# gizatechxyz/LuminAIR

Hardware: AMD Instinct MI355X
Metric: proofs/sec, 2^20-row Add trace (higher is better)
Workload: dtype u32 (M31/QM31 field arithmetic)

## Files before the change

### luminair_amd/csrc/fft_fixed.h

```cpp
#pragma once
#include "kernels.h"

namespace lmn {

bool launch_fft_fixed_pass(bool inverse, uint32_t* data, uint64_t col_stride, const uint32_t* src, uint64_t src_stride, int lo,
                           int rbits, int cb, int log_n, const TwPtrs& tw, uint32_t scale_log, int ncols, int cpb,
                           uint32_t h_off, int xcd_swizzle, bool zero_extended_top, lmn_stream_t s);
bool launch_interp_extend_fixed(uint32_t* coeffs, uint64_t coeff_stride, uint32_t* lde, uint64_t lde_stride, int log_n,
                                const TwPtrs& itw, const TwPtrs& tw_ext, int ncols, lmn_stream_t s);
bool launch_fft_rows_fixed(uint32_t* coeffs, uint64_t col_stride, const uint32_t* rows, uint64_t n_rows, int ncols, int log_n,
                           const PadRow& pad, uint32_t* bad_flag, uint32_t bad_value, const TwPtrs& itw, lmn_stream_t s);

}
```

### luminair_amd/csrc/fft_fixed.hip

```cpp
#include "fft_fixed.h"

#include <algorithm>

#include "issue_phases.h"
#include "launch_util.h"

namespace lmn {

LMN_HD constexpr uint32_t fx_pad(uint32_t e) { return e + (e >> 5); }

#if !defined(LMN_EMU) && !defined(LMN_BATCH)
#define LMN_BOUNDS(n) __launch_bounds__(n)
#else
#define LMN_BOUNDS(n)
#endif

struct GTile {
#if defined(__HIP_DEVICE_COMPILE__) && !defined(LMN_EMU)
  __amdgpu_buffer_rsrc_t r;
#else
  uint32_t* p;
#endif
};
LMN_D GTile gtile(const uint32_t* p) {
// ... 110 lines not shown
        d[k] = a[k] - x[k];
        d2[k] = d[k] + P31;
      }
      LMN_PHASE_PORT0();
#pragma unroll
      for (int k = 0; k < NB; ++k) {
        const int j = ((k >> r) << (r + 1)) | (k & ((1 << r) - 1));
        v[j] = u[k] < u2[k] ? u[k] : u2[k];
        v[j | (1 << r)] = d[k] < d2[k] ? d[k] : d2[k];
      }
    }
  }
  LMN_PHASE_ANY();
}

template <int R, int r, int HB>
LMN_D void fx_load_twiddles(uint32_t (&t2)[(1 << R) - 1], const uint32_t* const (&twd)[MAX_LOG], int layer0, uint32_t H,
                            uint32_t mhigh) {
  const uint32_t* __restrict__ t = twd[layer0 + r];
  const uint32_t hb = (H << (HB - r - 1)) + (mhigh << (R - 1 - r));
  LMN_ASSUME(hb < (1u << 28));
  fx_load_run<(1 << (R - 1 - r))>(t + hb, &t2[fx_tw_at<R>(r)]);
  if constexpr (r + 1 < R) fx_load_twiddles<R, r + 1, HB>(t2, twd, layer0, H, mhigh);
}

LMN_D uint32_t m_rot(uint32_t x, uint32_t e) {
#if defined(__HIP_DEVICE_COMPILE__) && !defined(LMN_EMU)
  return __builtin_amdgcn_alignbit(x, x + x, 32u - e) & P31;
#else
  return (uint32_t)((((uint64_t)x << e) | ((uint64_t)x >> (31u - e))) & P31);
#endif
}

template <int RBITS_, int CB_, bool LO0_>
struct FxShape {
  static constexpr int RBITS = RBITS_, CB = CB_, TB = RBITS_ + CB_;
  static constexpr bool LO0 = LO0_;
  static constexpr int NT = 1 << (TB - 4);
  static constexpr int NST = (RBITS + 3) / 4;
  static constexpr int R(int k) {
    int f = 0, r = 0;
    for (int i = 0; i <= k; ++i) {
      r = (RBITS - f + (NST - i) - 1) / (NST - i);
      f += r;
    }
    return r;
  }
  static constexpr int F(int k) {
    int f = 0;
    for (int i = 0; i < k; ++i) f += R(i);
    return f;
  }
  static constexpr uint32_t LDS_WORDS = (1u << TB) + ((1u << TB) >> 5) + 1u;
};

template <int R, bool INV, int P, class S, bool FG, bool TG, bool KEEP, bool ZX = false>
LMN_D void fx_stage(const uint32_t* sm_in, uint32_t* sm_out, uint32_t* tdst, const uint32_t* tsrc,
                    int lo, uint32_t H, const uint32_t* const (&twd)[MAX_LOG], uint32_t scale_log, uint32_t* keep, uint32_t tid) {
  constexpr int TB = S::TB, CB = S::CB, RBITS = S::RBITS;
  constexpr bool LO0 = S::LO0;
  constexpr uint32_t NG = 1u << (TB - R);
  constexpr uint32_t NT = (uint32_t)S::NT;
  constexpr int ITER = (int)(NG / NT);
  constexpr int L0 = P - CB;
  constexpr uint32_t cmask = (1u << CB) - 1u;
  static_assert(NG >= NT && P >= CB && P + R <= TB, "stage outside the tile");
#pragma unroll
  for (int it = 0; it < ITER; ++it) {
    const uint32_t g = tid + (uint32_t)it * NT;
    const uint32_t e0 = ((g >> P) << (P + R)) | (g & ((1u << P) - 1u));
    const uint32_t mhigh = e0 >> (P + R);
    uint32_t t2[(1 << R) - 1];
    fx_load_twiddles<R, 0, RBITS - L0>(t2, twd, (LO0 ? 0 : lo) + L0, H, mhigh);
    uint32_t v[1 << R];
    const uint32_t off0 = LO0 ? e0 : (((e0 >> CB) << lo) + (e0 & cmask));
    LMN_ASSUME(off0 < 0x10000000u);
    const int gshift = LO0 ? P : (P - CB + lo);
    if constexpr (FG) {
      if constexpr (LO0 && P == 0 && R >= 2) {
        fx_load_run<(1 << R)>(tsrc + e0, v);
      } else if constexpr (ZX) {
        static_assert(!INV && P + R == TB, "zero extension: forward transform, top stage");
        const GTile gt = gtile(tsrc);
#pragma unroll
        for (int j = 0; j < (1 << (R - 1)); ++j) {
          v[j] = gtile_load(gt, off0, (uint32_t)j << gshift);
          v[j + (1 << (R - 1))] = v[j];
        }
      } else {
        const GTile gt = gtile(tsrc);
#pragma unroll
        for (int j = 0; j < (1 << R); ++j) v[j] = gtile_load(gt, off0, (uint32_t)j << gshift);
      }
    } else {
      const uint32_t pb = fx_pad(e0);
#pragma unroll
      for (int j = 0; j < (1 << R); ++j) v[j] = sm_in[pb + fx_pad((uint32_t)j << P)];
    }
    fx_butterflies<R, INV, ZX>(v, t2);
    if constexpr (TG) {
      if constexpr (INV) {
        if (scale_log != 0u) {
#pragma unroll
          for (int j = 0; j < (1 << R); ++j) v[j] = m_rot(v[j], scale_log);
        }
      }
      if constexpr (LO0 && P == 0 && R >= 2) {
#if !defined(LMN_EMU)
// ... 36 lines not shown
}

struct TwD {
  const uint32_t* l[MAX_LOG];
};
static TwD doubled(const TwPtrs& tw) {
  TwD t{};
  for (int i = 0; i < MAX_LOG; ++i) t.l[i] = tw.d[i];
  return t;
}

template <bool INV, int RBITS, int CB, bool LO0, bool ZX = false>
LMN_KERNEL LMN_BOUNDS((FxShape<RBITS, CB, LO0>::NT))
k_fft_fx(uint32_t* data, uint64_t col_stride, const uint32_t* src, uint64_t src_stride, int lo_arg, TwD tw, uint32_t scale_log,
         int ncols, int cpb, uint32_t h_off, int xcd_swizzle) {
  using S = FxShape<RBITS, CB, LO0>;
  LMN_DYN_SMEM(uint32_t, sm);
  const int lo = LO0 ? 0 : lo_arg;
  uint32_t tile = blockIdx.x;
  if (xcd_swizzle && (gridDim.x & 7u) == 0u) tile = (blockIdx.x & 7u) * (gridDim.x >> 3) + (blockIdx.x >> 3);
  const uint32_t q = tile & ((1u << (lo - CB)) - 1u);
  const uint32_t Hl = tile >> (lo - CB);
  const uint64_t base = ((uint64_t)Hl << (lo + RBITS)) + ((uint64_t)q << CB);
  const uint32_t H = Hl + h_off;
  for (int cc = 0; cc < cpb; ++cc) {
    const int c = (int)blockIdx.y * cpb + cc;
    if (c >= ncols) break;
    uint32_t* col = data + (uint64_t)c * col_stride + base;
    const uint32_t* scol = src + (uint64_t)c * src_stride + base;
    fx_steps<S, INV, 0, true, true, false, ZX>(sm, sm, col, scol, lo, H, tw.l, scale_log, nullptr, threadIdx.x);
  }
}

template <int RBITS>
LMN_KERNEL LMN_BOUNDS((FxShape<RBITS, 4, false>::NT))
k_fft_interp_extend_fx(uint32_t* coeffs, uint64_t coeff_stride, uint32_t* lde, uint64_t lde_stride, TwD itw, TwD tw,
                       uint32_t scale_log) {
  using S = FxShape<RBITS, 4, false>;
  constexpr int LO = 12;
  LMN_DYN_SMEM(uint32_t, sm);
  uint32_t* A = sm;
  uint32_t* B = sm + S::LDS_WORDS;
  uint32_t tile = blockIdx.x;
  if ((gridDim.x & 7u) == 0u) tile = (blockIdx.x & 7u) * (gridDim.x >> 3) + (blockIdx.x >> 3);
  const uint64_t base = (uint64_t)tile << 4;
  const uint64_t n_words = 1ull << (LO + RBITS);
  uint32_t* ccol = coeffs + (uint64_t)blockIdx.y * coeff_stride + base;
  uint32_t* lcol = lde + (uint64_t)blockIdx.y * lde_stride + base;
  fx_steps<S, true, 0, true, true, true>(B, B, ccol, ccol, LO, 0u, itw.l, scale_log, A, threadIdx.x);
  for (uint32_t h = 0; h < 2; ++h)
    fx_steps<S, false, 0, false, true, false>(A, B, lcol + h * n_words, nullptr, LO, h, tw.l, 0u, nullptr, threadIdx.x);
}

template <int COLS>
LMN_KERNEL LMN_BOUNDS((COLS / 2) * 256)
k_fft_rows_fx(uint32_t* coeffs, uint64_t col_stride, const uint32_t* __restrict__ rows, uint64_t n_rows, int ncols, PadRow pad,
              uint32_t* __restrict__ bad_flag, uint32_t bad_value, TwD itw, uint32_t n_groups) {
  using S = FxShape<12, 0, true>;
  constexpr uint32_t NT = (uint32_t)S::NT, TILE = 1u << 12, GROUPS = COLS / 2;
  static_assert(NT == 256, "one lane group per tile");
  LMN_DYN_SMEM(uint32_t, sm);
  uint32_t tile = blockIdx.x / n_groups, ygrp = blockIdx.x % n_groups;
  if ((gridDim.x & 7u) == 0u && ((gridDim.x / n_groups) & 7u) == 0u) {
    const uint32_t x = blockIdx.x & 7u, sq = blockIdx.x >> 3;
    tile = (sq / n_groups) * 8u + x;
    ygrp = sq % n_groups;
  }
  const int c0 = (int)ygrp * COLS;
  const int ncb = ncols - c0 < COLS ? ncols - c0 : COLS;
  const uint64_t row0 = (uint64_t)tile << 12;
  {
    constexpr int BATCH = 8;
    constexpr uint32_t CELLS = TILE * COLS, STEP = GROUPS * NT;
    for (uint32_t k0 = threadIdx.x; k0 < CELLS; k0 += BATCH * STEP) {
      uint32_t v[BATCH];
#pragma unroll
      for (int j = 0; j < BATCH; ++j) {
        const uint32_t k = k0 + (uint32_t)j * STEP;
        const uint32_t r = k / COLS, c = k % COLS;
        const uint64_t gr = row0 + r;
        v[j] = 0u;
        if ((int)c < ncb) v[j] = gr < n_rows ? rows[gr * (uint64_t)ncols + (uint32_t)c0 + c] : pad.v[(uint32_t)c0 + c];
      }
#pragma unroll
      for (int j = 0; j < BATCH; ++j) {
        const uint32_t k = k0 + (uint32_t)j * STEP;
        const uint32_t r = k / COLS, c = k % COLS;
        if (v[j] >= P31) *bad_flag = bad_value;
        if ((int)c < ncb) sm[c * S::LDS_WORDS + fx_pad(r)] = v[j];
      }
    }
  }
  __syncthreads();
#if defined(__HIP_DEVICE_COMPILE__) && !defined(LMN_EMU)
  const uint32_t grp = __builtin_amdgcn_readfirstlane(threadIdx.x / NT);
#else
  const uint32_t grp = threadIdx.x / NT;
#endif
  const uint32_t tid = threadIdx.x % NT;
  for (int round = 0; round * (int)GROUPS < COLS; ++round) {
    const int cl = round * (int)GROUPS + (int)grp;
    const bool active = cl < ncb;
    uint32_t* t = sm + (uint32_t)(active ? cl : 0) * S::LDS_WORDS;
    uint32_t* col = coeffs + (uint64_t)(c0 + (active ? cl : 0)) * col_stride + row0;
    fx_steps<S, true, 0, false, true, false>(t, t, col, nullptr, 0, tile, itw.l, 0u, nullptr, tid, active);
  }
}

template <int COLS>
static void launch_rows_fx(uint32_t* coeffs, uint64_t col_stride, const uint32_t* rows, uint64_t n_rows, int ncols, int log_n,
                           const PadRow& pad, uint32_t* bad_flag, uint32_t bad_value, const TwPtrs& itw, lmn_stream_t s) {
  using S = FxShape<12, 0, true>;
  const size_t smem = (size_t)4 * COLS * S::LDS_WORDS;
  const uint32_t n_groups = (uint32_t)((ncols + COLS - 1) / COLS);
#if !defined(LMN_EMU) && !defined(LMN_BATCH)
  if (smem > 64 * 1024) allow_big_lds((const void*)k_fft_rows_fx<COLS>, 160 * 1024);
#endif
  LMN_LAUNCH((k_fft_rows_fx<COLS>), dim3((1u << (log_n - 12)) * n_groups), dim3((COLS / 2) * 256), smem, s, coeffs, col_stride,
             rows, n_rows, ncols, pad, bad_flag, bad_value, doubled(itw), n_groups);
}

bool launch_fft_rows_fixed(uint32_t* coeffs, uint64_t col_stride, const uint32_t* rows, uint64_t n_rows, int ncols, int log_n,
                           const PadRow& pad, uint32_t* bad_flag, uint32_t bad_value, const TwPtrs& itw, lmn_stream_t s) {
  static const bool off = env_set("LMN_NO_FFT_FIXED");
  if (off || !itw.d[0] || log_n < 13 || ncols < 1 || ncols > 32) return false;
  const int cols = env_int("LMN_ROWS_FX_COLS", 8);
  if (cols == 4)
    launch_rows_fx<4>(coeffs, col_stride, rows, n_rows, ncols, log_n, pad, bad_flag, bad_value, itw, s);
  else
    launch_rows_fx<8>(coeffs, col_stride, rows, n_rows, ncols, log_n, pad, bad_flag, bad_value, itw, s);
  return true;
}

template <bool INV, int RBITS, int CB, bool LO0, bool ZX = false>
static void launch_fx(uint32_t* data, uint64_t col_stride, const uint32_t* src, uint64_t src_stride, int lo, int log_n,
                      const TwPtrs& tw, uint32_t scale_log, int ncols, int cpb, uint32_t h_off, int xcd, lmn_stream_t s) {
  using S = FxShape<RBITS, CB, LO0>;
  const unsigned tiles = 1u << (log_n - S::TB);
  const size_t smem = (size_t)4 * S::LDS_WORDS;
#if !defined(LMN_EMU) && !defined(LMN_BATCH)
  if (smem > 64 * 1024) allow_big_lds((const void*)k_fft_fx<INV, RBITS, CB, LO0, ZX>, 160 * 1024);
#endif
  LMN_LAUNCH((k_fft_fx<INV, RBITS, CB, LO0, ZX>), dim3(tiles, (unsigned)((ncols + cpb - 1) / cpb)), dim3(S::NT), smem, s, data,
             col_stride, src, src_stride, lo, doubled(tw), scale_log, ncols, cpb, h_off, xcd);
}

template <bool INV>
static bool dispatch_fx(uint32_t* data, uint64_t col_stride, const uint32_t* src, uint64_t src_stride, int lo, int rbits, int cb,
                        int log_n, const TwPtrs& tw, uint32_t scale_log, int ncols, int cpb, uint32_t h_off, int xcd,
                        bool zext, lmn_stream_t s) {
#define LMN_FX_CASE(RB, CBV, L0V)                                                                                            \
  if constexpr (!INV && !L0V) {                                                                                              \
    if (zext) {                                                                                                              \
      launch_fx<INV, RB, CBV, L0V, true>(data, col_stride, src, src_stride, lo, log_n, tw, scale_log, ncols, cpb, h_off, xcd, \
                                         s);                                                                                 \
      return true;                                                                                                           \
    }                                                                                                                        \
  }                                                                                                                          \
  if (zext) return false;                                                                                                    \
  launch_fx<INV, RB, CBV, L0V>(data, col_stride, src, src_stride, lo, log_n, tw, scale_log, ncols, cpb, h_off, xcd, s);      \
  return true
  if (lo == 0 && cb == 0) {
    if (rbits == 12) { LMN_FX_CASE(12, 0, true); }
// ... 3 lines not shown
    switch (rbits) {
      case 5: LMN_FX_CASE(5, 5, false);
      case 6: LMN_FX_CASE(6, 5, false);
      case 7: LMN_FX_CASE(7, 5, false);
      default: return false;
    }
  }
  if (cb == 4 && lo >= 4) {
    switch (rbits) {
      case 6: LMN_FX_CASE(6, 4, false);
      case 7: LMN_FX_CASE(7, 4, false);
      case 8: LMN_FX_CASE(8, 4, false);
      case 9: LMN_FX_CASE(9, 4, false);
      case 10: LMN_FX_CASE(10, 4, false);
      default: return false;
    }
  }
  return false;
#undef LMN_FX_CASE
}

bool launch_fft_fixed_pass(bool inverse, uint32_t* data, uint64_t col_stride, const uint32_t* src, uint64_t src_stride, int lo,
                           int rbits, int cb, int log_n, const TwPtrs& tw, uint32_t scale_log, int ncols, int cpb,
                           uint32_t h_off, int xcd_swizzle, bool zero_extended_top, lmn_stream_t s) {
  static const bool off = env_set("LMN_NO_FFT_FIXED");
  if (off || !tw.d[0]) return false;
  if (zero_extended_top && (inverse || lo + rbits != log_n)) return false;
  return inverse ? dispatch_fx<true>(data, col_stride, src, src_stride, lo, rbits, cb, log_n, tw, scale_log, ncols, cpb, h_off,
                                     xcd_swizzle, false, s)
                 : dispatch_fx<false>(data, col_stride, src, src_stride, lo, rbits, cb, log_n, tw, scale_log, ncols, cpb, h_off,
                                      xcd_swizzle, zero_extended_top, s);
}

template <int RBITS>
static void launch_ie(uint32_t* coeffs, uint64_t coeff_stride, uint32_t* lde, uint64_t lde_stride, const TwPtrs& itw,
                      const TwPtrs& tw_ext, uint32_t scale_log, int ncols, lmn_stream_t s) {
  using S = FxShape<RBITS, 4, false>;
  const size_t smem = (size_t)8 * S::LDS_WORDS;
#if !defined(LMN_EMU) && !defined(LMN_BATCH)
  if (smem > 64 * 1024) allow_big_lds((const void*)k_fft_interp_extend_fx<RBITS>, 160 * 1024);
#endif
  LMN_LAUNCH((k_fft_interp_extend_fx<RBITS>), dim3(1u << (12 - 4), (unsigned)ncols), dim3(S::NT), smem, s, coeffs, coeff_stride,
             lde, lde_stride, doubled(itw), doubled(tw_ext), scale_log);
}

bool launch_interp_extend_fixed(uint32_t* coeffs, uint64_t coeff_stride, uint32_t* lde, uint64_t lde_stride, int log_n,
                                const TwPtrs& itw, const TwPtrs& tw_ext, int ncols, lmn_stream_t s) {
  static const bool off = env_set("LMN_NO_FFT_FIXED");
  if (off || !itw.d[0] || !tw_ext.d[0]) return false;
  const uint32_t scale_log = (uint32_t)((31 - (log_n % 31)) % 31);
  switch (log_n - 12) {
    case 6: launch_ie<6>(coeffs, coeff_stride, lde, lde_stride, itw, tw_ext, scale_log, ncols, s); return true;
    case 7: launch_ie<7>(coeffs, coeff_stride, lde, lde_stride, itw, tw_ext, scale_log, ncols, s); return true;
    case 8: launch_ie<8>(coeffs, coeff_stride, lde, lde_stride, itw, tw_ext, scale_log, ncols, s); return true;
    case 9: launch_ie<9>(coeffs, coeff_stride, lde, lde_stride, itw, tw_ext, scale_log, ncols, s); return true;
    default: return false;
  }
}

}
```

### luminair_amd/csrc/kernels.h

```cpp
#pragma once
#include "blake2s.h"
#include "field.h"

namespace lmn {

constexpr int MAX_LOG = 30;

struct TwPtrs {
  const uint32_t* l[MAX_LOG];
  const uint32_t* d[MAX_LOG];
};

struct PadRow {
  uint32_t v[32];
};
void launch_transpose_pad(const uint32_t* rows, uint64_t n_rows, int ncols, int log_size, uint32_t* cols,
                          const PadRow& pad, uint32_t* bad_flag , lmn_stream_t s);
void launch_transpose_pad_rows(const uint32_t* rows, uint64_t n_rows, int ncols, int log_size, uint32_t* cols,
                               uint64_t out_stride, uint64_t blk_row0, uint64_t blk_rows, const PadRow& pad, uint32_t* bad_flag,
                               lmn_stream_t s,
                               uint32_t bad_value = 1u );
constexpr int CHUNK_ROWS = 256;
constexpr int CHUNK_MAX_COLS = 30;
void launch_rows_chunk(const uint32_t* chunk, uint64_t r0, uint64_t n, int ncols, uint32_t* cols, uint64_t stride,
                       const PadRow& pad, uint32_t* bad_word, lmn_stream_t s);

int launch_ifft(uint32_t* dst, uint64_t dst_stride, const uint32_t* src, uint64_t src_stride, int ncols, int log_n,
                const TwPtrs& itw, lmn_stream_t s);
int launch_fft(uint32_t* dst, uint64_t dst_stride, const uint32_t* src, uint64_t src_stride, int log_src, int ncols,
               int log_n, const TwPtrs& tw, lmn_stream_t s);
bool fft_interp_extend_supported(int log_n);
int launch_interp_extend(uint32_t* coeffs, uint64_t coeff_stride, const uint32_t* evals, uint64_t evals_stride, uint32_t* lde,
                         uint64_t lde_stride, int ncols, int log_n, const TwPtrs& itw, const TwPtrs& tw_ext, lmn_stream_t s);
struct PadRow;
bool launch_interp_extend_rows(uint32_t* coeffs, uint64_t coeff_stride, const uint32_t* rows, uint64_t n_rows, const PadRow& pad,
                               uint32_t* bad_flag, uint32_t bad_value, uint32_t* lde, uint64_t lde_stride, int ncols, int log_n,
                               const TwPtrs& itw, const TwPtrs& tw_ext, lmn_stream_t s);
int launch_fft_block(uint32_t* dst, uint64_t dst_stride, const uint32_t* src, uint64_t src_stride, int log_src, int ncols,
                     int log_n, int log_blocks, uint32_t block, const TwPtrs& tw, lmn_stream_t s);
struct PackSel {
  uint32_t blk[8][2];
};
void launch_pack_blocks(const uint32_t* src, uint64_t src_stride, uint32_t* dst, uint32_t block_rows, int ncols, int nsel,
                        int world, const PackSel& sel, lmn_stream_t s);
void launch_unpack_blocks(const uint32_t* packed, uint32_t* cols, uint64_t col_stride, uint32_t block_rows, int ncols, int world,
                          lmn_stream_t s);
void launch_fft_simple(uint32_t* data, uint64_t col_stride, int ncols, int log_n, const TwPtrs& tw, bool inverse,
                       lmn_stream_t s);
void launch_extend(const uint32_t* src, uint64_t src_stride, int log_src, uint32_t* dst, uint64_t dst_stride,
                   int log_dst, int ncols, lmn_stream_t s);

void launch_bit_reverse(uint32_t* data, uint64_t col_stride, int ncols, int log_n, lmn_stream_t s);
int decompose_num_blocks(int log_n);
void launch_decompose(const uint32_t* f, int log_n, uint32_t* g, QM31* lambda_out, QM31* scratch, lmn_stream_t s);

void launch_merkle_layer(const uint32_t* prev, const uint32_t* const* cols, int ncols, uint32_t size, uint32_t* out,
                         lmn_stream_t s);

struct DevChannel {
  uint32_t digest[8];
  uint32_t n_sent;
  uint32_t variant;
};
void launch_chan_mix_root_draw(DevChannel* ch, const uint32_t* root, QM31* out_alpha, uint32_t* root_copy,
                               lmn_stream_t s);

constexpr int CHAN_N_ELEMS = 5;
// ... 290 lines not shown
```

### luminair_amd/csrc/kernels_fft.hip

```cpp
#include "kernels_common.h"

namespace lmn {

constexpr int FFT_MAX_STAGES = 4;
struct FftStagePlan {
  int lo, hi, cb;
  int nst;
  int first[FFT_MAX_STAGES];
  int R[FFT_MAX_STAGES];
  int xcd_swizzle;
};

LMN_HD uint32_t fft_lds_pad(uint32_t e) { return e + (e >> 5); }

template <int N>
LMN_D void m_mul_phased(const uint32_t (&x)[N], const uint32_t (&w)[N], uint32_t (&out)[N]) {
  uint64_t pr[N];
  uint32_t hi[N], s[N], s2[N];
  LMN_PHASE_PORT0();
#pragma unroll
  for (int k = 0; k < N; ++k) pr[k] = (uint64_t)x[k] * (uint64_t)w[k];
#pragma unroll
  for (int k = 0; k < N; ++k) hi[k] = (uint32_t)(pr[k] >> 31);
  LMN_PHASE_ANY();
// ... 305 lines not shown
    const uint32_t scale_log = scale == 1u ? 0u : (uint32_t)__builtin_ctz(scale);
    if (launch_fft_fixed_pass(INV, data, col_stride, psrc, pstride, p.lo, rbits, p.cb, log_n, tw, scale_log, ncols, cpb,
                              block_index << (log_n - p.hi), pl.xcd_swizzle, !full, s))
      return;
  }
  unsigned gy = (unsigned)((ncols + cpb - 1) / cpb);
  const int threads = (int)std::min<uint32_t>(TPB, std::max<uint32_t>(64u, tile_elems >> 4));
  LMN_LAUNCH(k_fft_staged<INV>, dim3(tiles, gy), dim3(threads), smem, s, data, col_stride, psrc, pstride, plen, pl, tw,
             scale, ncols, cpb, block_index << (log_n - p.hi));
}

template <bool INV>
static int run_fft(uint32_t* data, uint64_t col_stride, const uint32_t* src, uint64_t src_stride, int log_src,
                    int ncols, int log_n, const TwPtrs& tw, lmn_stream_t s, uint32_t block_index = 0) {
  if (log_n < 1) throw LmnError(-100, "fft: log_n < 1");
  FftPass passes[8];
  int np = plan_passes(log_n, passes);
  for (int k = 0; k < np; ++k) {
    const FftPass& p = INV ? passes[k] : passes[np - 1 - k];
    bool last = INV && k == np - 1;
    uint32_t scale = last ? inv_pow2(log_n) : 1u;
    const uint32_t* psrc = k == 0 ? src : data;
    uint64_t pstride = k == 0 ? src_stride : col_stride;
    uint64_t plen = k == 0 ? (1ull << log_src) : (1ull << log_n);
    launch_staged_pass<INV>(data, col_stride, psrc, pstride, plen, p, log_n, tw, scale, ncols, s, block_index);
  }
  return np;
}

bool fft_interp_extend_supported(int log_n) {
  static const bool off = env_set("LMN_NO_FFT_FUSION");
  return !off && log_n > FFT_LOW_BITS && log_n - FFT_LOW_BITS <= FFT_HIGH_BITS - 1;
}
static void interp_extend_tail(uint32_t* coeffs, uint64_t coeff_stride, uint32_t* lde, uint64_t lde_stride, int ncols, int log_n,
                               const TwPtrs& itw, const TwPtrs& tw_ext, lmn_stream_t s) {
  const FftPass low{0, FFT_LOW_BITS, 0};
  FftStagePlan pl{};
  pl.lo = FFT_LOW_BITS;
  pl.hi = log_n;
  pl.cb = FFT_HIGH_CB;
  split_stages(pl);
  pl.xcd_swizzle = 1;
  const uint32_t tile_elems = 1u << (log_n - FFT_LOW_BITS + FFT_HIGH_CB);
  const size_t smem = (size_t)8 * (tile_elems + (tile_elems >> 5) + 1);
  const unsigned tiles = 1u << (FFT_LOW_BITS - FFT_HIGH_CB);
  int cpb = 1;
  const int threads = (int)std::min<uint32_t>(TPB, std::max<uint32_t>(64u, tile_elems >> 4));
#if !defined(LMN_EMU) && !defined(LMN_BATCH)
  if (smem > 64 * 1024) allow_big_lds((const void*)k_fft_interp_extend, 160 * 1024);
#endif
  if (!launch_interp_extend_fixed(coeffs, coeff_stride, lde, lde_stride, log_n, itw, tw_ext, ncols, s))
    LMN_LAUNCH(k_fft_interp_extend, dim3(tiles, (unsigned)((ncols + cpb - 1) / cpb)), dim3(threads), smem, s, coeffs,
               coeff_stride, coeffs, coeff_stride, lde, lde_stride, pl, itw, tw_ext, inv_pow2(log_n), ncols, cpb);
  launch_staged_pass<false>(lde, lde_stride, lde, lde_stride, 2ull << log_n, low, log_n + 1, tw_ext, 1u, ncols, s);
}

int launch_interp_extend(uint32_t* coeffs, uint64_t coeff_stride, const uint32_t* evals, uint64_t evals_stride, uint32_t* lde,
                         uint64_t lde_stride, int ncols, int log_n, const TwPtrs& itw, const TwPtrs& tw_ext, lmn_stream_t s) {
  if (!fft_interp_extend_supported(log_n)) throw LmnError(-100, "interp_extend: unsupported size");
  const FftPass low{0, FFT_LOW_BITS, 0};
  launch_staged_pass<true>(coeffs, coeff_stride, evals, evals_stride, 1ull << log_n, low, log_n, itw, 1u, ncols, s);
  interp_extend_tail(coeffs, coeff_stride, lde, lde_stride, ncols, log_n, itw, tw_ext, s);
  return 3;
}

bool launch_interp_extend_rows(uint32_t* coeffs, uint64_t coeff_stride, const uint32_t* rows, uint64_t n_rows, const PadRow& pad,
                               uint32_t* bad_flag, uint32_t bad_value, uint32_t* lde, uint64_t lde_stride, int ncols, int log_n,
                               const TwPtrs& itw, const TwPtrs& tw_ext, lmn_stream_t s) {
  static_assert(FFT_LOW_BITS == 12, "k_fft_rows_fx is the 12-layer contiguous pass");
  if (!fft_interp_extend_supported(log_n)) return false;
  if (!launch_fft_rows_fixed(coeffs, coeff_stride, rows, n_rows, ncols, log_n, pad, bad_flag, bad_value, itw, s)) return false;
  interp_extend_tail(coeffs, coeff_stride, lde, lde_stride, ncols, log_n, itw, tw_ext, s);
  return true;
}

int launch_ifft(uint32_t* dst, uint64_t dst_stride, const uint32_t* src, uint64_t src_stride, int ncols, int log_n,
                const TwPtrs& itw, lmn_stream_t s) {
  return run_fft<true>(dst, dst_stride, src, src_stride, log_n, ncols, log_n, itw, s);
}
int launch_fft(uint32_t* dst, uint64_t dst_stride, const uint32_t* src, uint64_t src_stride, int log_src, int ncols,
               int log_n, const TwPtrs& tw, lmn_stream_t s) {
  return run_fft<false>(dst, dst_stride, src, src_stride, log_src, ncols, log_n, tw, s);
}

template <int G>
LMN_KERNEL k_fft_top_block(uint32_t* __restrict__ dst, uint64_t dst_stride, const uint32_t* __restrict__ src,
                           uint64_t src_stride, uint64_t src_len, int log_n, uint32_t block, TwPtrs tw) {
  const uint64_t S = 1ull << (log_n - G);
  const uint64_t t = (uint64_t)blockIdx.x * blockDim.x + threadIdx.x;
  if (t >= S) return;
  const uint32_t* scol = src + (uint64_t)blockIdx.y * src_stride;
  uint32_t v[1 << G];
#pragma unroll
  for (int c = 0; c < (1 << G); ++c) {
    const uint64_t idx = (uint64_t)c * S + t;
    v[c] = idx < src_len ? scol[idx] : 0u;
  }
#pragma unroll
  for (int k = G - 1; k >= 0; --k) {
    const uint32_t* __restrict__ tl = tw.l[log_n - G + k];
#pragma unroll
    for (int c = 0; c < (1 << G); ++c) {
      if (c & (1 << k)) continue;
      const uint32_t w = tl[c >> (k + 1)];
      const uint32_t a = v[c], x = m_mul(v[c | (1 << k)], w);
// ... 131 lines not shown
```

### luminair_amd/csrc/phase_trace.cpp

```cpp
#include "prove_run.h"

namespace lmn {

void Context::run_preprocessed(ProofRun& r) {
  LMN_RUN_ALIASES(r);
  const lmn_settings* settings = r.settings;
  for (auto& ti : infos) {
    Instance ci{};
    ci.spec = ti.spec;
    ci.log_size = ti.log_size;
    inst.push_back(ci);
  }
  {
    uint32_t present = 0;
    const lmn_lut* lut_of[3] = {nullptr, nullptr, nullptr};
    for (auto& ti : infos) {
      if (ti.spec->kind == LMN_KIND_SIN_LOOKUP) present |= LMN_LOOKUP_SIN;
      if (ti.spec->kind == LMN_KIND_EXP2_LOOKUP) present |= LMN_LOOKUP_EXP2;
      if (ti.spec->kind == LMN_KIND_LOG2_LOOKUP) present |= LMN_LOOKUP_LOG2;
      if (ti.spec->kind == LMN_KIND_RANGE_CHECK_LOOKUP) present |= LMN_LOOKUP_RANGE_CHECK;
    }
    if (settings && (settings->has_lookups & ~present))
      throw LmnError(LMN_ERR_INVALID_ARGUMENT, "settings announce a lookup whose table is not in the pie");
    if (settings && settings->n_luts) {
// ... 49 lines not shown
void Context::run_main_trace(ProofRun& r) {
  LMN_RUN_ALIASES(r);
  uint32_t* d_bad = bad_flag_;
  if (++bad_epoch_ < 2u) bad_epoch_ = 2u;
  const uint32_t bad_mark = shard_.active ? 1u : bad_epoch_;
  const uint32_t* h_bad = nullptr;
  bool any_rows_front = false;
  {
    StageTimer st(this, log, stream_, C_TRANSPOSE);
    for (size_t t = 0; t < infos.size(); ++t) {
      auto& ti = infos[t];
      uint64_t n = 1ull << ti.log_size;
      const bool rows_front = shard_rows_front(ti.log_size);
      const uint64_t nb = rows_front ? n >> shard_.g : n, blk0 = rows_front ? (uint64_t)shard_.rank * nb : 0;
      const uint64_t up0 = std::min<uint64_t>(blk0, ti.n_rows), up1 = std::min<uint64_t>(blk0 + nb, ti.n_rows);
      if (ti.cols_on_device) {
        inst[t].trace_evals = const_cast<uint32_t*>(ti.rows);
        inst[t].rows_n = ti.n_rows;
        proof.claim[ti.spec->kind] = ti.log_size;
        continue;
      }
      const uint32_t* d_rows = ti.rows;
      if (!ti.on_device) {
        uint32_t* stg = arena_.alloc_words(std::max<uint64_t>(up1 - up0, 1) * ti.spec->n_cols);
        if (up1 > up0) lmn_h2d(stg, ti.rows + up0 * ti.spec->n_cols, (up1 - up0) * ti.spec->n_cols * 4, stream_);
        d_rows = stg - up0 * ti.spec->n_cols;
      }
      PadRow pad{};
      if (ti.spec->is_last_col >= 0) pad.v[ti.spec->is_last_col] = 1u;
      for (int k = 0; k < ti.spec->n_pad; ++k) pad.v[ti.spec->pad_col[k]] = ti.spec->pad_val[k];
      inst[t].rows_dev = d_rows;
      inst[t].rows_n = ti.n_rows;
      inst[t].pad = pad;
      const bool try_fused = env_int("LMN_ROWS_FUSION", 0) != 0 && !shard_.active && lb == 1 && ti.spec->n_pre == 0 &&
                             fft_interp_extend_supported(ti.log_size) &&
                             ti.log_size >= std::max(13, env_int("LMN_ROWS_FUSION_MIN_LOG", 18)) && !env_set("LMN_NO_FFT_FIXED");
      if (try_fused) {
        inst[t].trace_evals = nullptr;
      } else {
        uint32_t* evals = arena_.alloc_words((size_t)ti.spec->n_cols * nb);
        launch_transpose_pad_rows(d_rows, ti.n_rows, ti.spec->n_cols, ti.log_size, evals, nb, blk0, nb, pad, d_bad, stream_, bad_mark);
        inst[t].trace_evals = evals;
      }
      inst[t].rows_sharded = rows_front;
      any_rows_front = any_rows_front || rows_front;
      proof.claim[ti.spec->kind] = ti.log_size;
    }
  }
  {
    StageTimer st(this, log, stream_, C_MAIN_COMMIT);
    int off = 0;
    for (auto& ci : inst) {
      uint64_t n = 1ull << ci.log_size;
      int nc = ci.spec->n_cols;
      uint32_t* coeffs = arena_.alloc_words((size_t)nc * n);
      CommitOut co;
      bool fused = false;
      if (!ci.trace_evals) {
        uint32_t* lde = arena_.alloc_words((size_t)nc * 2 * n);
        {
          StageTimer t(this, log, stream_, C_FFT);
          fused = launch_interp_extend_rows(coeffs, n, ci.rows_dev, ci.rows_n, ci.pad, d_bad, bad_mark, lde, 2 * n, nc, ci.log_size,
                                            itw(ci.log_size), tw(ci.log_size + 1), stream_);
        }
        if (fused) {
          timings.fft_launches += 3;
          timings.fft_bytes += (uint64_t)nc * 20ull * n;
          timings.fft_butterflies += (uint64_t)nc * (n / 2) * (uint64_t)ci.log_size + (uint64_t)nc * n * (uint64_t)ci.log_size;
          co.lde = lde;
          co.stride = 2 * n;
        } else {
          throw LmnError(LMN_ERR_INTERNAL, "main trace: no row pass for a size run_main_trace had chosen it for");
        }
      }
      if (!fused) co = interpolate_for_commit(coeffs, ci.trace_evals, nc, ci.log_size, -1, ci.rows_sharded);
      ci.main_start = off;
      off += nc;
      for (int c = 0; c < nc; ++c)
        tree1.cols.push_back({ci.log_size, coeffs + (uint64_t)c * n, co.lde ? co.lde + (uint64_t)c * co.stride : nullptr,
                              co.sharded, co.owner_of(c)});
    }
    for (int k = 0; k < n_slots; ++k)
      if (proof.claim[k] >= 0) channel.mix_u64((uint64_t)proof.claim[k]);
    r.bad_mark = bad_mark;
    if (r.dev_fs) {
      r.d_chan = (DevChannel*)arena_.alloc_bytes(sizeof(DevChannel));
      r.d_report = (DevReport*)arena_.alloc_bytes(sizeof(DevReport));
      ChanStep step{};
      step.kind = 1;
      memcpy(step.start.digest, channel.digest().w, 32);
      step.start.n_sent = 0;
      step.start.variant = (cfg.protocol_variant & LMN_PV_DRAW_CTR_U32) ? 1u : 0u;
      step.bad_word = d_bad;
      int sets[CHAN_N_ELEMS];
      const int n_draws = relation_draw_sets(cfg.protocol_variant, sets);
      if (n_draws < 1 || n_draws > CHAN_N_ELEMS) throw LmnError(LMN_ERR_INTERNAL, "relation draws: bad count");
      step.sets.n = n_draws;
      for (int i = 0; i < n_draws; ++i) step.sets.set[i] = sets[i];
      step.rep = r.d_report;
      lde_and_merkle(tree1, false, r.d_chan, &step);
      for (int i = 0; i < n_draws; ++i)
        if (sets[i] >= 0) elems.drawn[sets[i]] = true;
      hm.mark("main trace enqueued (device transcript)");
      return;
    }
    lde_and_merkle(tree1);
    uint32_t n_flags = 1;
    if (any_rows_front) {
// ... 27 lines not shown
```

### luminair_amd/roofline.py

```python
from __future__ import annotations

import json
import os
from typing import Dict, Optional

HBM_PEAK_GBS = 8000.0
BLAKE2S_PEAK_GCOMP = 63.8
BUTTERFLY_PEAK_G = 4800.0
N_SIMD, MAX_CLOCK_GHZ, ISSUE_PER_CLK_PER_SIMD = 1024, 2.4, 0.5
LANE_INSTR_PER_S = N_SIMD * MAX_CLOCK_GHZ * 1e9 * ISSUE_PER_CLK_PER_SIMD * 64
INSTR_PER_COMPRESSION, INSTR_PER_BUTTERFLY = 12 * 80 + 16, 11

KERNEL_FAMILIES = {
    "k_fft_fx": ("fft", ["k_fft_staged<false>", "k_fft_staged<true>", "k_fft_interp_extend", "k_fft_fx", "k_fft_interp_extend_fx"],
                 "fft_butterflies", BUTTERFLY_PEAK_G, "G butterflies/s", INSTR_PER_BUTTERFLY),
    "k_merkle_fused": ("merkle_fused", ["k_merkle_fused", "k_merkle_fused<0>", "k_merkle_fused<1>", "k_merkle_fused<2>",
                                        "k_merkle_fused<3>", "k_merkle_fused<4>"],
                       "merkle_fused_compressions", BLAKE2S_PEAK_GCOMP, "G Blake2s compressions/s", INSTR_PER_COMPRESSION),
}


PMC_ROUND = "r6"


def load_pmc(root: str):
    import glob
    import re
    import sys
    cur = os.path.join(root, "profiles", "%s_pmc_summary.json" % PMC_ROUND)
    older = sorted((p_ for p_ in glob.glob(os.path.join(root, "profiles", "r*_pmc_summary.json")) if p_ != cur),
                   key=lambda p_: int(re.search(r"r(\d+)_pmc_summary", p_).group(1)), reverse=True)
    for pth in [cur] + older:
        if not os.path.exists(pth):
            continue
        try:
            with open(pth) as f:
                kernels = json.load(f)["kernels"]
        except (OSError, ValueError, KeyError):
            continue
        name = "profiles/" + os.path.basename(pth)
        if pth != cur:
            sys.stderr.write("bench.py: WARNING: %s is missing; `traffic` comes from the STALE counter summary %s\n"
                             % (os.path.relpath(cur, root), name))
            name += " [STALE: counters of an earlier round's tree, this round's summary (%s) is missing]" % os.path.basename(cur)
        return kernels, name
    return {}, None

# ... 48 lines not shown
```

Measured before the change: 787.0.

## Shrink row-pass FFT to 10 layers and enable row fusion by default

The fused row-transpose plus inverse FFT kernel now does 10 layers per tile with one 64-lane wave per column instead of 12 layers with 256 threads per column. This cuts LDS per block and should raise occupancy. The two remaining low layers move into the strided interpolate/extend kernel through a split-word tile addressing mode (XB). The path that fuses the row pass into interpolation is also switched on by default for log sizes 18 to 20, which removes the separate transpose-pad and evals buffer. The cost is a more complex strided kernel with wider tiles, and a fallback to the unfused path for other sizes.

```diff
diff --git a/luminair_amd/csrc/fft_fixed.h b/luminair_amd/csrc/fft_fixed.h
--- a/luminair_amd/csrc/fft_fixed.h
+++ b/luminair_amd/csrc/fft_fixed.h
@@ -7,8 +7,9 @@
                            int rbits, int cb, int log_n, const TwPtrs& tw, uint32_t scale_log, int ncols, int cpb,
                            uint32_t h_off, int xcd_swizzle, bool zero_extended_top, lmn_stream_t s);
 bool launch_interp_extend_fixed(uint32_t* coeffs, uint64_t coeff_stride, uint32_t* lde, uint64_t lde_stride, int log_n,
-                                const TwPtrs& itw, const TwPtrs& tw_ext, int ncols, lmn_stream_t s);
+                                const TwPtrs& itw, const TwPtrs& tw_ext, int ncols, int layers_done, lmn_stream_t s);
 bool launch_fft_rows_fixed(uint32_t* coeffs, uint64_t col_stride, const uint32_t* rows, uint64_t n_rows, int ncols, int log_n,
                            const PadRow& pad, uint32_t* bad_flag, uint32_t bad_value, const TwPtrs& itw, lmn_stream_t s);
+bool fft_rows_fixed_supported(int log_n, int ncols);
 
 }
diff --git a/luminair_amd/csrc/fft_fixed.hip b/luminair_amd/csrc/fft_fixed.hip
--- a/luminair_amd/csrc/fft_fixed.hip
+++ b/luminair_amd/csrc/fft_fixed.hip
@@ -166,9 +166,10 @@
 #endif
 }
 
-template <int RBITS_, int CB_, bool LO0_>
+template <int RBITS_, int CB_, bool LO0_, int XB_ = 0>
 struct FxShape {
-  static constexpr int RBITS = RBITS_, CB = CB_, TB = RBITS_ + CB_;
+  static constexpr int RBITS = RBITS_, CB = CB_, TB = RBITS_ + CB_, XB = XB_;
+  static_assert(XB_ >= 0 && XB_ <= CB_ && !(LO0_ && XB_), "split word bits: strided tiles only");
   static constexpr bool LO0 = LO0_;
   static constexpr int NT = 1 << (TB - 4);
   static constexpr int NST = (RBITS + 3) / 4;
@@ -207,7 +208,11 @@
     uint32_t t2[(1 << R) - 1];
     fx_load_twiddles<R, 0, RBITS - L0>(t2, twd, (LO0 ? 0 : lo) + L0, H, mhigh);
     uint32_t v[1 << R];
-    const uint32_t off0 = LO0 ? e0 : (((e0 >> CB) << lo) + (e0 & cmask));
+    uint32_t off0 = LO0 ? e0 : (((e0 >> CB) << lo) + (e0 & cmask));
+    if constexpr (S::XB > 0) {
+      constexpr uint32_t wmask = (1u << (CB - S::XB)) - 1u;
+      off0 = ((e0 >> CB) << lo) + (((e0 & cmask) >> (CB - S::XB)) << (lo - S::XB)) + (e0 & wmask);
+    }
     LMN_ASSUME(off0 < 0x10000000u);
     const int gshift = LO0 ? P : (P - CB + lo);
     if constexpr (FG) {
@@ -310,33 +315,53 @@
   }
 }
 
+template <int RBITS, int XB, int CB>
+LMN_D void fx_interp_extend_tile(uint32_t* sm, uint32_t* coeffs, uint64_t coeff_stride, uint32_t* lde, uint64_t lde_stride,
+                                 const TwD& itw, const TwD& tw, uint32_t scale_log) {
+  using SI = FxShape<RBITS + XB, CB, false>;
+  using SF = FxShape<RBITS, CB + XB, false, XB>;
+  static_assert(SI::LDS_WORDS == SF::LDS_WORDS && SI::NT == SF::NT, "both halves share the tile");
+  constexpr int LO = 12;
+  uint32_t* A = sm;
+  uint32_t* B = sm + SI::LDS_WORDS;
+  uint32_t tile = blockIdx.x;
+  if ((gridDim.x & 7u) == 0u) tile = (blockIdx.x & 7u) * (gridDim.x >> 3) + (blockIdx.x >> 3);
+  const uint64_t base = (uint64_t)tile << CB;
+  const uint64_t n_words = 1ull << (LO + RBITS);
+  uint32_t* ccol = coeffs + (uint64_t)blockIdx.y * coeff_stride + base;
+  uint32_t* lcol = lde + (uint64_t)blockIdx.y * lde_stride + base;
+  fx_steps<SI, true, 0, true, true, true>(B, B, ccol, ccol, LO - XB, 0u, itw.l, scale_log, A, threadIdx.x);
+  for (uint32_t h = 0; h < 2; ++h)
+    fx_steps<SF, false, 0, false, true, false>(A, B, lcol + h * n_words, nullptr, LO, h, tw.l, 0u, nullptr, threadIdx.x);
+}
+
 template <int RBITS>
 LMN_KERNEL LMN_BOUNDS((FxShape<RBITS, 4, false>::NT))
 k_fft_interp_extend_fx(uint32_t* coeffs, uint64_t coeff_stride, uint32_t* lde, uint64_t lde_stride, TwD itw, TwD tw,
                        uint32_t scale_log) {
-  using S = FxShape<RBITS, 4, false>;
-  constexpr int LO = 12;
   LMN_DYN_SMEM(uint32_t, sm);
-  uint32_t* A = sm;
-  uint32_t* B = sm + S::LDS_WORDS;
-  uint32_t tile = blockIdx.x;
-  if ((gridDim.x & 7u) == 0u) tile = (blockIdx.x & 7u) * (gridDim.x >> 3) + (blockIdx.x >> 3);
-  const uint64_t base = (uint64_t)tile << 4;
-  const uint64_t n_words = 1ull << (LO + RBITS);
-  uint32_t* ccol = coeffs + (uint64_t)blockIdx.y * coeff_stride + base;
-  uint32_t* lcol = lde + (uint64_t)blockIdx.y * lde_stride + base;
-  fx_steps<S, true, 0, true, true, true>(B, B, ccol, ccol, LO, 0u, itw.l, scale_log, A, threadIdx.x);
-  for (uint32_t h = 0; h < 2; ++h)
-    fx_steps<S, false, 0, false, true, false>(A, B, lcol + h * n_words, nullptr, LO, h, tw.l, 0u, nullptr, threadIdx.x);
-}
-
-template <int COLS>
-LMN_KERNEL LMN_BOUNDS((COLS / 2) * 256)
+  fx_interp_extend_tile<RBITS, 0, 4>(sm, coeffs, coeff_stride, lde, lde_stride, itw, tw, scale_log);
+}
+
+constexpr int ROWS_FX_LAYERS = 10;
+template <int RBITS>
+LMN_KERNEL LMN_BOUNDS((FxShape<RBITS + 12 - ROWS_FX_LAYERS, 4, false>::NT))
+k_fft_interp_extend_rows_fx(uint32_t* coeffs, uint64_t coeff_stride, uint32_t* lde, uint64_t lde_stride, TwD itw, TwD tw,
+                            uint32_t scale_log) {
+  LMN_DYN_SMEM(uint32_t, sm);
+  fx_interp_extend_tile<RBITS, 12 - ROWS_FX_LAYERS, 4>(sm, coeffs, coeff_stride, lde, lde_stride, itw, tw, scale_log);
+}
+
+constexpr int ROWS_FX_COLS = 8;
+constexpr uint32_t ROWS_FX_COL_WORDS = FxShape<ROWS_FX_LAYERS, 0, true>::LDS_WORDS + 7u;
+static_assert(ROWS_FX_COL_WORDS % 64u == 40u, "column tiles 8 banks apart (mod 64, times an odd factor)");
+
+LMN_KERNEL LMN_BOUNDS(ROWS_FX_COLS * 64)
 k_fft_rows_fx(uint32_t* coeffs, uint64_t col_stride, const uint32_t* __restrict__ rows, uint64_t n_rows, int ncols, PadRow pad,
               uint32_t* __restrict__ bad_flag, uint32_t bad_value, TwD itw, uint32_t n_groups) {
-  using S = FxShape<12, 0, true>;
-  constexpr uint32_t NT = (uint32_t)S::NT, TILE = 1u << 12, GROUPS = COLS / 2;
-  static_assert(NT == 256, "one lane group per tile");
+  using S = FxShape<ROWS_FX_LAYERS, 0, true>;
+  constexpr uint32_t NT = (uint32_t)S::NT, TILE = 1u << ROWS_FX_LAYERS, COLS = ROWS_FX_COLS;
+  static_assert(NT == 64, "one wave per column");
   LMN_DYN_SMEM(uint32_t, sm);
   uint32_t tile = blockIdx.x / n_groups, ygrp = blockIdx.x % n_groups;
   if ((gridDim.x & 7u) == 0u && ((gridDim.x / n_groups) & 7u) == 0u) {
@@ -344,12 +369,12 @@
     tile = (sq / n_groups) * 8u + x;
     ygrp = sq % n_groups;
   }
-  const int c0 = (int)ygrp * COLS;
-  const int ncb = ncols - c0 < COLS ? ncols - c0 : COLS;
-  const uint64_t row0 = (uint64_t)tile << 12;
+  const int c0 = (int)ygrp * (int)COLS;
+  const int ncb = ncols - c0 < (int)COLS ? ncols - c0 : (int)COLS;
+  const uint64_t row0 = (uint64_t)tile << ROWS_FX_LAYERS;
   {
     constexpr int BATCH = 8;
-    constexpr uint32_t CELLS = TILE * COLS, STEP = GROUPS * NT;
+    constexpr uint32_t CELLS = TILE * COLS, STEP = COLS * NT;
     for (uint32_t k0 = threadIdx.x; k0 < CELLS; k0 += BATCH * STEP) {
       uint32_t v[BATCH];
 #pragma unroll
@@ -365,48 +390,37 @@
         const uint32_t k = k0 + (uint32_t)j * STEP;
         const uint32_t r = k / COLS, c = k % COLS;
         if (v[j] >= P31) *bad_flag = bad_value;
-        if ((int)c < ncb) sm[c * S::LDS_WORDS + fx_pad(r)] = v[j];
+        if ((int)c < ncb) sm[c * ROWS_FX_COL_WORDS + fx_pad(r)] = v[j];
       }
     }
   }
   __syncthreads();
 #if defined(__HIP_DEVICE_COMPILE__) && !defined(LMN_EMU)
-  const uint32_t grp = __builtin_amdgcn_readfirstlane(threadIdx.x / NT);
-#else
-  const uint32_t grp = threadIdx.x / NT;
-#endif
-  const uint32_t tid = threadIdx.x % NT;
-  for (int round = 0; round * (int)GROUPS < COLS; ++round) {
-    const int cl = round * (int)GROUPS + (int)grp;
-    const bool active = cl < ncb;
-    uint32_t* t = sm + (uint32_t)(active ? cl : 0) * S::LDS_WORDS;
-    uint32_t* col = coeffs + (uint64_t)(c0 + (active ? cl : 0)) * col_stride + row0;
-    fx_steps<S, true, 0, false, true, false>(t, t, col, nullptr, 0, tile, itw.l, 0u, nullptr, tid, active);
-  }
-}
-
-template <int COLS>
-static void launch_rows_fx(uint32_t* coeffs, uint64_t col_stride, const uint32_t* rows, uint64_t n_rows, int ncols, int log_n,
-                           const PadRow& pad, uint32_t* bad_flag, uint32_t bad_value, const TwPtrs& itw, lmn_stream_t s) {
-  using S = FxShape<12, 0, true>;
-  const size_t smem = (size_t)4 * COLS * S::LDS_WORDS;
-  const uint32_t n_groups = (uint32_t)((ncols + COLS - 1) / COLS);
-#if !defined(LMN_EMU) && !defined(LMN_BATCH)
-  if (smem > 64 * 1024) allow_big_lds((const void*)k_fft_rows_fx<COLS>, 160 * 1024);
-#endif
-  LMN_LAUNCH((k_fft_rows_fx<COLS>), dim3((1u << (log_n - 12)) * n_groups), dim3((COLS / 2) * 256), smem, s, coeffs, col_stride,
-             rows, n_rows, ncols, pad, bad_flag, bad_value, doubled(itw), n_groups);
+  const uint32_t cl = __builtin_amdgcn_readfirstlane(threadIdx.x / NT);
+#else
+  const uint32_t cl = threadIdx.x / NT;
+#endif
+  const bool active = (int)cl < ncb;
+  uint32_t* t = sm + (active ? cl : 0u) * ROWS_FX_COL_WORDS;
+  uint32_t* col = coeffs + (uint64_t)(c0 + (active ? (int)cl : 0)) * col_stride + row0;
+  fx_steps<S, true, 0, false, true, false>(t, t, col, nullptr, 0, tile, itw.l, 0u, nullptr, threadIdx.x % NT, active);
+}
+
+bool fft_rows_fixed_supported(int log_n, int ncols) {
+#if defined(LMN_BATCH)
+  return false;
+#else
+  return log_n >= 18 && log_n <= 20 && ncols >= 1 && ncols <= 32;
+#endif
 }
 
 bool launch_fft_rows_fixed(uint32_t* coeffs, uint64_t col_stride, const uint32_t* rows, uint64_t n_rows, int ncols, int log_n,
                            const PadRow& pad, uint32_t* bad_flag, uint32_t bad_value, const TwPtrs& itw, lmn_stream_t s) {
-  static const bool off = env_set("LMN_NO_FFT_FIXED");
-  if (off || !itw.d[0] || log_n < 13 || ncols < 1 || ncols > 32) return false;
-  const int cols = env_int("LMN_ROWS_FX_COLS", 8);
-  if (cols == 4)
-    launch_rows_fx<4>(coeffs, col_stride, rows, n_rows, ncols, log_n, pad, bad_flag, bad_value, itw, s);
-  else
-    launch_rows_fx<8>(coeffs, col_stride, rows, n_rows, ncols, log_n, pad, bad_flag, bad_value, itw, s);
+  if (!itw.d[0] || log_n < ROWS_FX_LAYERS || ncols < 1 || ncols > 32) return false;
+  const size_t smem = (size_t)4 * ROWS_FX_COLS * ROWS_FX_COL_WORDS;
+  const uint32_t n_groups = (uint32_t)((ncols + ROWS_FX_COLS - 1) / ROWS_FX_COLS);
+  LMN_LAUNCH(k_fft_rows_fx, dim3((1u << (log_n - ROWS_FX_LAYERS)) * n_groups), dim3(ROWS_FX_COLS * 64), smem, s, coeffs,
+             col_stride, rows, n_rows, ncols, pad, bad_flag, bad_value, doubled(itw), n_groups);
   return true;
 }
 
@@ -476,23 +490,42 @@
                                       xcd_swizzle, zero_extended_top, s);
 }
 
-template <int RBITS>
+template <int RBITS, bool ROWS = false>
 static void launch_ie(uint32_t* coeffs, uint64_t coeff_stride, uint32_t* lde, uint64_t lde_stride, const TwPtrs& itw,
                       const TwPtrs& tw_ext, uint32_t scale_log, int ncols, lmn_stream_t s) {
-  using S = FxShape<RBITS, 4, false>;
+  constexpr int XB = ROWS ? 12 - ROWS_FX_LAYERS : 0;
+  using S = FxShape<RBITS + XB, 4, false>;
   const size_t smem = (size_t)8 * S::LDS_WORDS;
+  const dim3 grid(1u << (12 - XB - 4), (unsigned)ncols), block(S::NT);
+  if constexpr (ROWS) {
 #if !defined(LMN_EMU) && !defined(LMN_BATCH)
-  if (smem > 64 * 1024) allow_big_lds((const void*)k_fft_interp_extend_fx<RBITS>, 160 * 1024);
-#endif
-  LMN_LAUNCH((k_fft_interp_extend_fx<RBITS>), dim3(1u << (12 - 4), (unsigned)ncols), dim3(S::NT), smem, s, coeffs, coeff_stride,
-             lde, lde_stride, doubled(itw), doubled(tw_ext), scale_log);
+    if (smem > 64 * 1024) allow_big_lds((const void*)k_fft_interp_extend_rows_fx<RBITS>, 160 * 1024);
+#endif
+    LMN_LAUNCH((k_fft_interp_extend_rows_fx<RBITS>), grid, block, smem, s, coeffs, coeff_stride, lde, lde_stride, doubled(itw),
+               doubled(tw_ext), scale_log);
+  } else {
+#if !defined(LMN_EMU) && !defined(LMN_BATCH)
+    if (smem > 64 * 1024) allow_big_lds((const void*)k_fft_interp_extend_fx<RBITS>, 160 * 1024);
+#endif
+    LMN_LAUNCH((k_fft_interp_extend_fx<RBITS>), grid, block, smem, s, coeffs, coeff_stride, lde, lde_stride, doubled(itw),
+               doubled(tw_ext), scale_log);
+  }
 }
 
 bool launch_interp_extend_fixed(uint32_t* coeffs, uint64_t coeff_stride, uint32_t* lde, uint64_t lde_stride, int log_n,
-                                const TwPtrs& itw, const TwPtrs& tw_ext, int ncols, lmn_stream_t s) {
+                                const TwPtrs& itw, const TwPtrs& tw_ext, int ncols, int layers_done, lmn_stream_t s) {
   static const bool off = env_set("LMN_NO_FFT_FIXED");
   if (off || !itw.d[0] || !tw_ext.d[0]) return false;
   const uint32_t scale_log = (uint32_t)((31 - (log_n % 31)) % 31);
+  if (layers_done == ROWS_FX_LAYERS) {
+    switch (log_n - 12) {
+      case 6: launch_ie<6, true>(coeffs, coeff_stride, lde, lde_stride, itw, tw_ext, scale_log, ncols, s); return true;
+      case 7: launch_ie<7, true>(coeffs, coeff_stride, lde, lde_stride, itw, tw_ext, scale_log, ncols, s); return true;
+      case 8: launch_ie<8, true>(coeffs, coeff_stride, lde, lde_stride, itw, tw_ext, scale_log, ncols, s); return true;
+      default: return false;
+    }
+  }
+  if (layers_done != 12) return false;
   switch (log_n - 12) {
     case 6: launch_ie<6>(coeffs, coeff_stride, lde, lde_stride, itw, tw_ext, scale_log, ncols, s); return true;
     case 7: launch_ie<7>(coeffs, coeff_stride, lde, lde_stride, itw, tw_ext, scale_log, ncols, s); return true;
diff --git a/luminair_amd/csrc/kernels.h b/luminair_amd/csrc/kernels.h
--- a/luminair_amd/csrc/kernels.h
+++ b/luminair_amd/csrc/kernels.h
@@ -33,6 +33,7 @@
 int launch_interp_extend(uint32_t* coeffs, uint64_t coeff_stride, const uint32_t* evals, uint64_t evals_stride, uint32_t* lde,
                          uint64_t lde_stride, int ncols, int log_n, const TwPtrs& itw, const TwPtrs& tw_ext, lmn_stream_t s);
 struct PadRow;
+bool fft_interp_extend_rows_supported(int log_n, int ncols);
 bool launch_interp_extend_rows(uint32_t* coeffs, uint64_t coeff_stride, const uint32_t* rows, uint64_t n_rows, const PadRow& pad,
                                uint32_t* bad_flag, uint32_t bad_value, uint32_t* lde, uint64_t lde_stride, int ncols, int log_n,
                                const TwPtrs& itw, const TwPtrs& tw_ext, lmn_stream_t s);
diff --git a/luminair_amd/csrc/kernels_fft.hip b/luminair_amd/csrc/kernels_fft.hip
--- a/luminair_amd/csrc/kernels_fft.hip
+++ b/luminair_amd/csrc/kernels_fft.hip
@@ -361,8 +361,8 @@
   static const bool off = env_set("LMN_NO_FFT_FUSION");
   return !off && log_n > FFT_LOW_BITS && log_n - FFT_LOW_BITS <= FFT_HIGH_BITS - 1;
 }
-static void interp_extend_tail(uint32_t* coeffs, uint64_t coeff_stride, uint32_t* lde, uint64_t lde_stride, int ncols, int log_n,
-                               const TwPtrs& itw, const TwPtrs& tw_ext, lmn_stream_t s) {
+static bool interp_extend_tail(uint32_t* coeffs, uint64_t coeff_stride, uint32_t* lde, uint64_t lde_stride, int ncols, int log_n,
+                               const TwPtrs& itw, const TwPtrs& tw_ext, lmn_stream_t s, int layers_done = FFT_LOW_BITS) {
   const FftPass low{0, FFT_LOW_BITS, 0};
   FftStagePlan pl{};
   pl.lo = FFT_LOW_BITS;
@@ -378,10 +378,13 @@
 #if !defined(LMN_EMU) && !defined(LMN_BATCH)
   if (smem > 64 * 1024) allow_big_lds((const void*)k_fft_interp_extend, 160 * 1024);
 #endif
-  if (!launch_interp_extend_fixed(coeffs, coeff_stride, lde, lde_stride, log_n, itw, tw_ext, ncols, s))
+  if (!launch_interp_extend_fixed(coeffs, coeff_stride, lde, lde_stride, log_n, itw, tw_ext, ncols, layers_done, s)) {
+    if (layers_done != FFT_LOW_BITS) return false;
     LMN_LAUNCH(k_fft_interp_extend, dim3(tiles, (unsigned)((ncols + cpb - 1) / cpb)), dim3(threads), smem, s, coeffs,
                coeff_stride, coeffs, coeff_stride, lde, lde_stride, pl, itw, tw_ext, inv_pow2(log_n), ncols, cpb);
+  }
   launch_staged_pass<false>(lde, lde_stride, lde, lde_stride, 2ull << log_n, low, log_n + 1, tw_ext, 1u, ncols, s);
+  return true;
 }
 
 int launch_interp_extend(uint32_t* coeffs, uint64_t coeff_stride, const uint32_t* evals, uint64_t evals_stride, uint32_t* lde,
@@ -393,13 +396,17 @@
   return 3;
 }
 
+bool fft_interp_extend_rows_supported(int log_n, int ncols) {
+  static const bool off = env_set("LMN_NO_FFT_FIXED");
+  return !off && fft_interp_extend_supported(log_n) && fft_rows_fixed_supported(log_n, ncols);
+}
 bool launch_interp_extend_rows(uint32_t* coeffs, uint64_t coeff_stride, const uint32_t* rows, uint64_t n_rows, const PadRow& pad,
                                uint32_t* bad_flag, uint32_t bad_value, uint32_t* lde, uint64_t lde_stride, int ncols, int log_n,
                                const TwPtrs& itw, const TwPtrs& tw_ext, lmn_stream_t s) {
-  static_assert(FFT_LOW_BITS == 12, "k_fft_rows_fx is the 12-layer contiguous pass");
-  if (!fft_interp_extend_supported(log_n)) return false;
+  if (!fft_interp_extend_rows_supported(log_n, ncols) || !itw.d[0] || !tw_ext.d[0]) return false;
   if (!launch_fft_rows_fixed(coeffs, coeff_stride, rows, n_rows, ncols, log_n, pad, bad_flag, bad_value, itw, s)) return false;
-  interp_extend_tail(coeffs, coeff_stride, lde, lde_stride, ncols, log_n, itw, tw_ext, s);
+  if (!interp_extend_tail(coeffs, coeff_stride, lde, lde_stride, ncols, log_n, itw, tw_ext, s, 10))
+    throw LmnError(-100, "interp_extend_rows: no strided pass behind the row pass");
   return true;
 }
 
diff --git a/luminair_amd/csrc/phase_trace.cpp b/luminair_amd/csrc/phase_trace.cpp
--- a/luminair_amd/csrc/phase_trace.cpp
+++ b/luminair_amd/csrc/phase_trace.cpp
@@ -105,9 +105,8 @@
       inst[t].rows_dev = d_rows;
       inst[t].rows_n = ti.n_rows;
       inst[t].pad = pad;
-      const bool try_fused = env_int("LMN_ROWS_FUSION", 0) != 0 && !shard_.active && lb == 1 && ti.spec->n_pre == 0 &&
-                             fft_interp_extend_supported(ti.log_size) &&
-                             ti.log_size >= std::max(13, env_int("LMN_ROWS_FUSION_MIN_LOG", 18)) && !env_set("LMN_NO_FFT_FIXED");
+      const bool try_fused = !shard_.active && lb == 1 && ti.spec->n_pre == 0 &&
+                             fft_interp_extend_rows_supported(ti.log_size, ti.spec->n_cols);
       if (try_fused) {
         inst[t].trace_evals = nullptr;
       } else {
@@ -128,25 +127,28 @@
       int nc = ci.spec->n_cols;
       uint32_t* coeffs = arena_.alloc_words((size_t)nc * n);
       CommitOut co;
-      bool fused = false;
+      bool done = false;
       if (!ci.trace_evals) {
         uint32_t* lde = arena_.alloc_words((size_t)nc * 2 * n);
         {
           StageTimer t(this, log, stream_, C_FFT);
-          fused = launch_interp_extend_rows(coeffs, n, ci.rows_dev, ci.rows_n, ci.pad, d_bad, bad_mark, lde, 2 * n, nc, ci.log_size,
+          done = launch_interp_extend_rows(coeffs, n, ci.rows_dev, ci.rows_n, ci.pad, d_bad, bad_mark, lde, 2 * n, nc, ci.log_size,
                                             itw(ci.log_size), tw(ci.log_size + 1), stream_);
+          if (!done) {
+            uint32_t* evals = arena_.alloc_words((size_t)nc * n);
+            launch_transpose_pad_rows(ci.rows_dev, ci.rows_n, nc, ci.log_size, evals, n, 0, n, ci.pad, d_bad, stream_, bad_mark);
+            launch_interp_extend(coeffs, n, evals, n, lde, 2 * n, nc, ci.log_size, itw(ci.log_size), tw(ci.log_size + 1), stream_);
+            ci.trace_evals = evals;
+            done = true;
+          }
         }
-        if (fused) {
-          timings.fft_launches += 3;
-          timings.fft_bytes += (uint64_t)nc * 20ull * n;
-          timings.fft_butterflies += (uint64_t)nc * (n / 2) * (uint64_t)ci.log_size + (uint64_t)nc * n * (uint64_t)ci.log_size;
-          co.lde = lde;
-          co.stride = 2 * n;
-        } else {
-          throw LmnError(LMN_ERR_INTERNAL, "main trace: no row pass for a size run_main_trace had chosen it for");
-        }
-      }
-      if (!fused) co = interpolate_for_commit(coeffs, ci.trace_evals, nc, ci.log_size, -1, ci.rows_sharded);
+        timings.fft_launches += 3;
+        timings.fft_bytes += (uint64_t)nc * 20ull * n;
+        timings.fft_butterflies += (uint64_t)nc * (n / 2) * (uint64_t)ci.log_size + (uint64_t)nc * n * (uint64_t)ci.log_size;
+        co.lde = lde;
+        co.stride = 2 * n;
+      }
+      if (!done) co = interpolate_for_commit(coeffs, ci.trace_evals, nc, ci.log_size, -1, ci.rows_sharded);
       ci.main_start = off;
       off += nc;
       for (int c = 0; c < nc; ++c)
diff --git a/luminair_amd/roofline.py b/luminair_amd/roofline.py
--- a/luminair_amd/roofline.py
+++ b/luminair_amd/roofline.py
@@ -12,7 +12,8 @@
 INSTR_PER_COMPRESSION, INSTR_PER_BUTTERFLY = 12 * 80 + 16, 11
 
 KERNEL_FAMILIES = {
-    "k_fft_fx": ("fft", ["k_fft_staged<false>", "k_fft_staged<true>", "k_fft_interp_extend", "k_fft_fx", "k_fft_interp_extend_fx"],
+    "k_fft_fx": ("fft", ["k_fft_staged<false>", "k_fft_staged<true>", "k_fft_interp_extend", "k_fft_fx", "k_fft_interp_extend_fx",
+                              "k_fft_rows_fx", "k_fft_interp_extend_rows_fx"],
                  "fft_butterflies", BUTTERFLY_PEAK_G, "G butterflies/s", INSTR_PER_BUTTERFLY),
     "k_merkle_fused": ("merkle_fused", ["k_merkle_fused", "k_merkle_fused<0>", "k_merkle_fused<1>", "k_merkle_fused<2>",
                                         "k_merkle_fused<3>", "k_merkle_fused<4>"],
```

Measured after the change: 788.9, median of 5. About the same (+0.2%).
